# Biomedical-Imaging-Group/MolecularDiffusion_MiViT

Measured on AMD Instinct MI355X. Metric: training image-sequences/sec, higher is better.
Workload: dtype bf16; 1 GPU; PSFNoise 32-frame 64x64 sequences, MiViT depth=4 dim=128 heads=4 hidden=256, linear frame embedding + regression token; train step = fwd + MSE + bwd + AdamW; per_gpu_batch=16384, global_batch=16384, frames=32, frame=64x64, parallelism=dp1, input_dtype=f32 frames resident in HBM

## Files before the change

### moleculardiffusion_mivit_amd/csrc/fused_bwd.hip

```cpp
#include "common.h"
#include "stream_prims.h"
#include <stdlib.h>
#include <algorithm>
#include <vector>
#include <stdio.h>
#include <type_traits>
#include "elem.h"

#define RC(call) do { int rc_ = (call); if (rc_) return rc_; } while (0)

namespace {

#ifdef MIVIT_WIDTH64
constexpr int E = 64, F = 128;
constexpr int LDE = E + 16, LDF = F + 16;
#else
constexpr int E = 128, F = 256;
constexpr int LDE = E + 16, LDF = F + 16;
#endif
constexpr int NW = 4, NT = NW * 64, R = 32;
constexpr int KS = E / 32, ET = E / 16;
constexpr int CPR = E / 8;
constexpr int RPP = NT / CPR, RPT = R / RPP;
constexpr int FW = F / NW, NTW = FW / 16;
// ... 242 lines not shown
#pragma unroll
                for (int nt = 0; nt < NTW; ++nt) {
                    dW1[nt][t] = mma(dhB[nt], xb, dW1[nt][t]);
                    dW2[t][nt] = mma(zb, hB[nt], dW2[t][nt]);
                }
                xb = xn; zb = zn;
            }
        }
        PT_MARK(4);
        barrier();
        PT_MARK(5);
        f32x4 dx[KT2][2];
#pragma unroll
        for (int kt = 0; kt < KT2; ++kt)
#pragma unroll
            for (int rt = 0; rt < 2; ++rt) dx[kt][rt] = zero;
        {
            auto wfrag = [&](int ks, int kt) {
                return tr_pair(W1i + (32 * ks + 4 * g + q) * LDE + EW * wave + 16 * kt + 4 * pp,
                               W1i + (32 * ks + 16 + 4 * g + q) * LDE + EW * wave + 16 * kt + 4 * pp);
            };
            const bf16 *dbase[2] = {DH + (4 * g + q) * R + ((g & 1) << 4) + 4 * pp, DH + (4 * g + q) * R + (((g & 1) ^ 1) << 4) + 4 * pp};
            auto dfrag = [&](int ks, int rt) { return tr_pair(dbase[rt] + 32 * ks * R, dbase[rt] + (32 * ks + 16) * R); };
            bf16x8 d0 = dfrag(0, 0), d1 = dfrag(0, 1);
            bf16x8 wf[KT2];
#pragma unroll
            for (int kt = 0; kt < KT2; ++kt) wf[kt] = wfrag(0, kt);
#pragma unroll
            for (int ks = 0; ks < FS; ++ks) {
                bf16x8 e0 = d0, e1 = d1, vf[KT2];
#pragma unroll
                for (int kt = 0; kt < KT2; ++kt) vf[kt] = wf[kt];
                if (ks < FS - 1) {
                    e0 = dfrag(ks + 1, 0); e1 = dfrag(ks + 1, 1);
#pragma unroll
                    for (int kt = 0; kt < KT2; ++kt) vf[kt] = wfrag(ks + 1, kt);
                }
#pragma unroll
                for (int kt = 0; kt < KT2; ++kt) { dx[kt][0] = mma(wf[kt], d0, dx[kt][0]); dx[kt][1] = mma(wf[kt], d1, dx[kt][1]); }
                d0 = e0; d1 = e1;
#pragma unroll
                for (int kt = 0; kt < KT2; ++kt) wf[kt] = vf[kt];
            }
        }
#pragma unroll
        for (int rt = 0; rt < 2; ++rt) {
            const int row = row0 + 16 * rt + cq;
#pragma unroll
            for (int kt = 0; kt < KT2; ++kt) {
                const int col = EW * wave + 16 * kt + 4 * g;
                const uint2 zr = *reinterpret_cast<const uint2 *>(DZ + (16 * rt + cq) * LDE + col);
                f32x4 o = dx[kt][rt];
                o[0] += elem_lo(zr.x); o[1] += elem_hi(zr.x);
                o[2] += elem_lo(zr.y); o[3] += elem_hi(zr.y);
                if (row < a.M) {
                    typedef __attribute__((ext_vector_type(4))) __bf16 bf16x4;
                    const bf16x4 ob = {(__bf16)o[0], (__bf16)o[1], (__bf16)o[2], (__bf16)o[3]};
                    *reinterpret_cast<bf16x4 *>(a.dx1 + (int64_t)row * E + col) = ob;
                }
            }
        }
        PT_MARK(6);
        barrier();
        PT_MARK(7);
    }
#ifdef MIVIT_PHASE_TIMING
    if (a.dbg && lane == 0)
        for (int k = 0; k < 8; ++k) a.dbg[((int64_t)blockIdx.x * NW + wave) * 8 + k] = pt[k];
#endif

    float *sl = a.slabs + (int64_t)blockIdx.x * SL_TOTAL;
#pragma unroll
    for (int nt = 0; nt < NTW; ++nt) {
#pragma unroll
        for (int t = 0; t < ET; ++t)
#pragma unroll
            for (int j = 0; j < 4; ++j) {
                sl[SL_W1 + (FW * wave + 16 * nt + 4 * g + j) * E + 16 * t + cq] = dW1[nt][t][j];
                sl[SL_W2 + (16 * t + 4 * g + j) * F + FW * wave + 16 * nt + cq] = dW2[t][nt][j];
            }
        const float s = x4_sum(db1[nt]);
        if (g == 0) sl[SL_B1 + FW * wave + 16 * nt + cq] = s;
    }
    __syncthreads();
    for (int i = tid; i < 3 * E; i += NT) {
        const int which = i / E, col = i - which * E, cc = col >> 3, e = col & 7;
        float s = 0.f;
        for (int rr = 0; rr < RPP; ++rr) s += cacc[(2 * which + (e >> 2)) * NT + cc + CPR * rr][e & 3];
        sl[(which == 0 ? SL_G2 : which == 1 ? SL_BE2 : SL_B2) + col] = s;
    }
}

#ifndef MIVIT_WIDTH64
constexpr int NW8 = 8, NT8 = NW8 * 64, NH = NT8 / 2;

template <int ACT>
__global__ __launch_bounds__(NT8) void mlp_block_bwd8_kernel(const MlpBwdArgs a) {
    extern __shared__ __attribute__((aligned(16))) unsigned char smem[];
    bf16 *W1i = reinterpret_cast<bf16 *>(smem + OFF_W1);
    bf16 *X = reinterpret_cast<bf16 *>(smem + OFF_X), *DZ = reinterpret_cast<bf16 *>(smem + OFF_DZ), *DH = reinterpret_cast<bf16 *>(smem + OFF_DH);
    float *b1f = reinterpret_cast<float *>(smem + OFF_VEC);
    f32x4 *cacc = reinterpret_cast<f32x4 *>(smem + OFF_ACC);
    uint4 *stg = reinterpret_cast<uint4 *>(smem + OFF_STG);
    float *rst = reinterpret_cast<float *>(smem + OFF_RST);
    const int tid = threadIdx.x, lane = tid & 63, wave = tid >> 6, g = lane >> 4, cq = lane & 15, q = cq >> 2, pp = cq & 3;
    const f32x4 zero = {0.f, 0.f, 0.f, 0.f};
    const int wave_u = __builtin_amdgcn_readfirstlane(wave);
    const bool ew = wave_u < 4;
    const int th = tid & (NH - 1), wh = wave_u & 3;
    const unsigned stg_a = __builtin_amdgcn_readfirstlane(lds_addr(stg)) + wh * 1024u, rst_a = __builtin_amdgcn_readfirstlane(lds_addr(rst)) + wh * 256u;

    static_assert((F * (E / 8)) % (4 * NT8) == 0, "W1 staging batches");
    for (int i0 = tid; i0 < F * (E / 8); i0 += 4 * NT8) {
        uint4 v0, v1, v2, v3;
        {
            const int i = i0, n = i / (E / 8), cc = i - n * (E / 8);
            v0 = *reinterpret_cast<const uint4 *>(a.W1 + (int64_t)n * E + cc * 8);
        }
        { const int i = i0 + NT8, n = i / (E / 8), cc = i - n * (E / 8); v1 = *reinterpret_cast<const uint4 *>(a.W1 + (int64_t)n * E + cc * 8); }
        { const int i = i0 + 2 * NT8, n = i / (E / 8), cc = i - n * (E / 8); v2 = *reinterpret_cast<const uint4 *>(a.W1 + (int64_t)n * E + cc * 8); }
        { const int i = i0 + 3 * NT8, n = i / (E / 8), cc = i - n * (E / 8); v3 = *reinterpret_cast<const uint4 *>(a.W1 + (int64_t)n * E + cc * 8); }
        { const int i = i0, n = i / (E / 8), cc = i - n * (E / 8); *reinterpret_cast<uint4 *>(W1i + n * LDE + cc * 8) = v0; }
        { const int i = i0 + NT8, n = i / (E / 8), cc = i - n * (E / 8); *reinterpret_cast<uint4 *>(W1i + n * LDE + cc * 8) = v1; }
        { const int i = i0 + 2 * NT8, n = i / (E / 8), cc = i - n * (E / 8); *reinterpret_cast<uint4 *>(W1i + n * LDE + cc * 8) = v2; }
        { const int i = i0 + 3 * NT8, n = i / (E / 8), cc = i - n * (E / 8); *reinterpret_cast<uint4 *>(W1i + n * LDE + cc * 8) = v3; }
    }
    for (int n = tid; n < F; n += NT8) b1f[n] = a.b1[n];
    for (int i = tid; i < E; i += NT8) { b1f[F + i] = a.gamma2[i]; b1f[F + E + i] = a.gamma1[i]; b1f[F + 2 * E + i] = a.beta1[i]; }
    bf16x8 w2f[2][4];
#pragma unroll
    for (int nt = 0; nt < 2; ++nt) {
        const int n = 32 * wave + 16 * nt + cq;
#pragma unroll
        for (int ks = 0; ks < 4; ++ks) {
            bf16x8 t;
#pragma unroll
            for (int e = 0; e < 8; ++e) t[e] = __builtin_bit_cast(__bf16, a.W2[(int64_t)(ks * 32 + 8 * g + e) * F + n].v);
            w2f[nt][ks] = t;
        }
    }
    typedef __attribute__((address_space(3))) const float lds_cf;
    if (ew) {
#pragma unroll
        for (int i = 0; i < 6; ++i) cacc[i * NH + th] = f32x4{0.f, 0.f, 0.f, 0.f};
    }
    f32x4 dW1[2][8], dW2[8][2];
#pragma unroll
    for (int i = 0; i < 2; ++i)
#pragma unroll
        for (int j = 0; j < 8; ++j) { dW1[i][j] = zero; dW2[j][i] = zero; }
    float db1[2] = {0.f, 0.f};
    __syncthreads();

    const int ntiles = (a.M + R - 1) / R;
    int tile = blockIdx.x;
    auto prefetch = [&](int t, int r0, int c) {
#pragma unroll
        for (int i = 0; i < 2; ++i) {
            const int row = min(t * R + r0 + 16 * i, a.M - 1);
            const unsigned o = ((unsigned)row * E + 8 * c) * 2u;
            if (ew) {
                dma16_sbase(a.dy, o, stg_a + (2 * i + 0) * NH * 16u);
                dma16_sbase(a.n2, o, stg_a + (2 * i + 1) * NH * 16u);
                dma4_sbase(a.rstd2, (unsigned)row * 4u, rst_a + i * NH * 4u);
            } else {
                dma16_sbase(a.n1, o, stg_a + (4 + i) * NH * 16u);
            }
        }
    };
    if (tile < ntiles) prefetch(tile, th >> 4, th & 15);
    bool first = true;
#ifdef MIVIT_PHASE_TIMING
    unsigned long long pt[8] = {0, 0, 0, 0, 0, 0, 0, 0}, pt_last = __builtin_amdgcn_s_memtime();
#endif
    for (; tile < ntiles; tile += gridDim.x) {
        const int row0 = tile * R;
        int thv = th;
        asm volatile("" : "+v"(thv));
        const int c = thv & 15, r0 = thv >> 4;
        lds_cf *gam2 = (lds_cf *)(b1f + F + 8 * c), *gam1 = (lds_cf *)(b1f + F + E + 8 * c), *bet1 = (lds_cf *)(b1f + F + 2 * E + 8 * c);
        if (first) wait_vm<0>(); else wait_vm<2>();
        first = false;
        PT_MARK(0);
        if (ew) {
            float sg[8], sb[8], sz[8];
#pragma unroll
            for (int e = 0; e < 8; ++e) sg[e] = sb[e] = sz[e] = 0.f;
            typedef __attribute__((address_space(3))) const f32x4 lds_cf4;
            const f32x4 g2a = *(lds_cf4 *)(gam2), g2b = *(lds_cf4 *)(gam2 + 4);
            const float g2v[8] = {g2a[0], g2a[1], g2a[2], g2a[3], g2b[0], g2b[1], g2b[2], g2b[3]};
#pragma unroll
            for (int i = 0; i < 2; ++i) {
                float d[8], nh[8];
                const bool ok = row0 + r0 + 16 * i < a.M;
                const uint4 pdy = keep_if(stg[(2 * i + 0) * NH + thv], ok), pn2 = stg[(2 * i + 1) * NH + thv];
                unpack8(pdy, d); unpack8(pn2, nh);
                float s1 = 0.f, s2 = 0.f;
#pragma unroll
                for (int e = 0; e < 8; ++e) {
                    sg[e] += d[e] * nh[e]; sb[e] += d[e];
                    d[e] *= g2v[e];
                    s1 += d[e]; s2 += d[e] * nh[e];
                }
                s1 = g16_sum(s1) * (1.f / E); s2 = g16_sum(s2) * (1.f / E);
                const float prs = __uint_as_float(__float_as_uint(rst[i * NH + thv]) & (ok ? 0xffffffffu : 0u));
                float dz[8];
#pragma unroll
                for (int e = 0; e < 8; ++e) { dz[e] = prs * (d[e] - s1 - nh[e] * s2); sz[e] += dz[e]; }
                store16(DZ + (r0 + 16 * i) * LDE + 8 * c, dz);
                __builtin_amdgcn_sched_barrier(0);
            }
            {
                f32x4 ca[3];
#pragma unroll
                for (int k = 0; k < 3; ++k) ca[k] = cacc[k * NH + thv];
                __builtin_amdgcn_sched_barrier(0);
                cacc[0 * NH + thv] = ca[0] + f32x4{sg[0], sg[1], sg[2], sg[3]}; cacc[1 * NH + thv] = ca[1] + f32x4{sg[4], sg[5], sg[6], sg[7]};
                cacc[2 * NH + thv] = ca[2] + f32x4{sb[0], sb[1], sb[2], sb[3]};
                __builtin_amdgcn_sched_barrier(0);
#pragma unroll
                for (int k = 0; k < 3; ++k) ca[k] = cacc[(3 + k) * NH + thv];
                __builtin_amdgcn_sched_barrier(0);
                cacc[3 * NH + thv] = ca[0] + f32x4{sb[4], sb[5], sb[6], sb[7]};
                cacc[4 * NH + thv] = ca[1] + f32x4{sz[0], sz[1], sz[2], sz[3]}; cacc[5 * NH + thv] = ca[2] + f32x4{sz[4], sz[5], sz[6], sz[7]};
            }
        } else {
            typedef __attribute__((address_space(3))) const f32x4 lds_cf4;
            const f32x4 g1a = *(lds_cf4 *)(gam1), g1b = *(lds_cf4 *)(gam1 + 4), b1a = *(lds_cf4 *)(bet1), b1b = *(lds_cf4 *)(bet1 + 4);
            const float g1v[8] = {g1a[0], g1a[1], g1a[2], g1a[3], g1b[0], g1b[1], g1b[2], g1b[3]};
            const float b1v[8] = {b1a[0], b1a[1], b1a[2], b1a[3], b1b[0], b1b[1], b1b[2], b1b[3]};
#pragma unroll
            for (int i = 0; i < 2; ++i) {
                const bool ok = row0 + r0 + 16 * i < a.M;
                const uint4 pn1 = keep_if(stg[(4 + i) * NH + thv], ok);
                float x1v[8];
                unpack8(pn1, x1v);
#pragma unroll
                for (int e = 0; e < 8; ++e) x1v[e] = ok ? x1v[e] * g1v[e] + b1v[e] : 0.f;
                store16(X + (r0 + 16 * i) * LDE + 8 * c, x1v);
            }
        }
        asm volatile("s_waitcnt lgkmcnt(0)" ::: "memory");
        PT_MARK(1);
        prefetch(min(tile + (int)gridDim.x, ntiles - 1), r0, c);
        barrier();
        PT_MARK(2);
        bf16x8 hB[2], dhB[2];
        {
            typedef __attribute__((ext_vector_type(4))) __bf16 bf16x4;
            const int dst_lane = (32 * wave + cq) * R + 4 * g, dst_sw0 = (q & 1) << 4, dst_sw1 = ((q & 1) ^ 1) << 4;
            bf16x4 hlo[2], dlo[2];
#pragma unroll
            for (int rt = 0; rt < 2; ++rt) {
                f32x4 u[2], dh[2];
#pragma unroll
                for (int n2 = 0; n2 < 2; ++n2) {
                    const float bv = b1f[32 * wave + 16 * n2 + cq];
                    u[n2] = f32x4{bv, bv, bv, bv}; dh[n2] = zero;
                }
#pragma unroll
                for (int ks = 0; ks < 4; ++ks) {
                    const bf16x8 xa = lds_frag(X + (16 * rt + cq) * LDE + ks * 32 + 8 * g);
                    const bf16x8 za = lds_frag(DZ + (16 * rt + cq) * LDE + ks * 32 + 8 * g);
#pragma unroll
                    for (int n2 = 0; n2 < 2; ++n2) {
                        u[n2] = mma(xa, lds_frag(W1i + (32 * wave + 16 * n2 + cq) * LDE + ks * 32 + 8 * g), u[n2]);
                        dh[n2] = mma(za, w2f[n2][ks], dh[n2]);
                    }
                }
#pragma unroll
                for (int n2 = 0; n2 < 2; ++n2) {
#pragma unroll
                    for (int j = 0; j < 4; ++j) {
                        const float uu = u[n2][j];
                        dh[n2][j] *= act_bwd(ACT, ACT == MIVIT_ACT_GELU ? uu : act_fwd(ACT, uu));
                        u[n2][j] = act_fwd(ACT, uu);
                        db1[n2] += dh[n2][j];
                    }
                    const bf16x4 hb = {(__bf16)u[n2][0], (__bf16)u[n2][1], (__bf16)u[n2][2], (__bf16)u[n2][3]};
                    const bf16x4 db = {(__bf16)dh[n2][0], (__bf16)dh[n2][1], (__bf16)dh[n2][2], (__bf16)dh[n2][3]};
                    *reinterpret_cast<bf16x4 *>(DH + dst_lane + (rt ? dst_sw1 : dst_sw0) + 16 * n2 * R) = db;
                    if (rt == 0) { hlo[n2] = hb; dlo[n2] = db; }
                    else {
                        struct { bf16x4 lo, hi; } ph = {hlo[n2], hb}, pd = {dlo[n2], db};
                        hB[n2] = __builtin_bit_cast(bf16x8, ph);
                        dhB[n2] = __builtin_bit_cast(bf16x8, pd);
                    }
                }
            }
        }
        PT_MARK(3);
        {
            bf16x8 xb = tr_pair(X + (4 * g + q) * LDE + 4 * pp, X + (16 + 4 * g + q) * LDE + 4 * pp);
            bf16x8 zb = tr_pair(DZ + (4 * g + q) * LDE + 4 * pp, DZ + (16 + 4 * g + q) * LDE + 4 * pp);
#pragma unroll
            for (int t = 0; t < 8; ++t) {
                bf16x8 xn = xb, zn = zb;
                if (t < 7) {
                    xn = tr_pair(X + (4 * g + q) * LDE + 16 * (t + 1) + 4 * pp, X + (16 + 4 * g + q) * LDE + 16 * (t + 1) + 4 * pp);
                    zn = tr_pair(DZ + (4 * g + q) * LDE + 16 * (t + 1) + 4 * pp, DZ + (16 + 4 * g + q) * LDE + 16 * (t + 1) + 4 * pp);
                }
#pragma unroll
                for (int nt = 0; nt < 2; ++nt) {
                    dW1[nt][t] = mma(dhB[nt], xb, dW1[nt][t]);
                    dW2[t][nt] = mma(zb, hB[nt], dW2[t][nt]);
                }
                xb = xn; zb = zn;
            }
        }
        PT_MARK(4);
        barrier();
        PT_MARK(5);
        f32x4 dx[2] = {zero, zero};
        {
            auto wfrag = [&](int ks) {
                return tr_pair(W1i + (32 * ks + 4 * g + q) * LDE + 16 * wave + 4 * pp, W1i + (32 * ks + 16 + 4 * g + q) * LDE + 16 * wave + 4 * pp);
            };
            const bf16 *dbase[2] = {DH + (4 * g + q) * R + ((g & 1) << 4) + 4 * pp, DH + (4 * g + q) * R + (((g & 1) ^ 1) << 4) + 4 * pp};
            auto dfrag = [&](int ks, int rt) { return tr_pair(dbase[rt] + 32 * ks * R, dbase[rt] + (32 * ks + 16) * R); };
            bf16x8 d0 = dfrag(0, 0), d1 = dfrag(0, 1), w0 = wfrag(0);
#pragma unroll
            for (int ks = 0; ks < 8; ++ks) {
                bf16x8 e0 = d0, e1 = d1, v0 = w0;
                if (ks < 7) { e0 = dfrag(ks + 1, 0); e1 = dfrag(ks + 1, 1); v0 = wfrag(ks + 1); }
                dx[0] = mma(w0, d0, dx[0]); dx[1] = mma(w0, d1, dx[1]);
                d0 = e0; d1 = e1; w0 = v0;
            }
        }
#pragma unroll
        for (int rt = 0; rt < 2; ++rt) {
            const int row = row0 + 16 * rt + cq, col = 16 * wave + 4 * g;
            const uint2 zr = *reinterpret_cast<const uint2 *>(DZ + (16 * rt + cq) * LDE + col);
            f32x4 o = dx[rt];
            o[0] += elem_lo(zr.x); o[1] += elem_hi(zr.x);
            o[2] += elem_lo(zr.y); o[3] += elem_hi(zr.y);
            if (row < a.M) {
                typedef __attribute__((ext_vector_type(4))) __bf16 bf16x4;
                const bf16x4 ob = {(__bf16)o[0], (__bf16)o[1], (__bf16)o[2], (__bf16)o[3]};
                *reinterpret_cast<bf16x4 *>(a.dx1 + (int64_t)row * E + col) = ob;
            }
        }
        PT_MARK(6);
        barrier();
        PT_MARK(7);
    }
#ifdef MIVIT_PHASE_TIMING
    if (a.dbg && lane == 0)
        for (int kk = 0; kk < 8; ++kk) a.dbg[((int64_t)blockIdx.x * NW8 + wave) * 8 + kk] = pt[kk];
#endif

    float *sl = a.slabs + (int64_t)blockIdx.x * SL_TOTAL;
#pragma unroll
    for (int nt = 0; nt < 2; ++nt) {
#pragma unroll
        for (int t = 0; t < 8; ++t)
#pragma unroll
            for (int j = 0; j < 4; ++j) {
                sl[SL_W1 + (32 * wave + 16 * nt + 4 * g + j) * E + 16 * t + cq] = dW1[nt][t][j];
                sl[SL_W2 + (16 * t + 4 * g + j) * F + 32 * wave + 16 * nt + cq] = dW2[t][nt][j];
            }
        const float sv = x4_sum(db1[nt]);
        if (g == 0) sl[SL_B1 + 32 * wave + 16 * nt + cq] = sv;
    }
    __syncthreads();
    for (int i = tid; i < 3 * E; i += NT8) {
        const int which = i / E, col = i - which * E, cc = col >> 3, e = col & 7;
        float sv = 0.f;
        for (int rr = 0; rr < 16; ++rr) sv += cacc[(2 * which + (e >> 2)) * NH + cc + 16 * rr][e & 3];
        sl[(which == 0 ? SL_G2 : which == 1 ? SL_BE2 : SL_B2) + col] = sv;
    }
}

#endif

constexpr int AO_OFF_DZ = 0, AO_OFF_CT = AO_OFF_DZ + R * LDE * 2, AO_OFF_STG = AO_OFF_CT + R * LDE * 2;
constexpr int AO_OFF_RED = AO_OFF_STG + 3 * RPT * NT * 16;
constexpr int AO_OFF_RST = AO_OFF_RED + NW * 3 * E * 4;
constexpr int AO_LDS = AO_OFF_RST + RPT * NT * 4;
constexpr int AO_SL_W = 0, AO_SL_B = E * E, AO_SL_G = AO_SL_B + E, AO_SL_BE = AO_SL_G + E, AO_SL_TOTAL = AO_SL_BE + E;
struct AttnOutBwdArgs {
    const bf16 *dy, *n1; const float *rstd1, *gamma1;
    const bf16 *ctx, *Wo;
    int M;
    bf16 *dz1, *dctx;
    float *slabs;
};

__global__ __launch_bounds__(NT, 2) void attn_out_bwd_kernel(const AttnOutBwdArgs a) {
    extern __shared__ __attribute__((aligned(16))) unsigned char smem[];
    bf16 *DZ = reinterpret_cast<bf16 *>(smem + AO_OFF_DZ), *CT = reinterpret_cast<bf16 *>(smem + AO_OFF_CT);
    uint4 *stg = reinterpret_cast<uint4 *>(smem + AO_OFF_STG);
    float *red = reinterpret_cast<float *>(smem + AO_OFF_RED);
    float *rst = reinterpret_cast<float *>(smem + AO_OFF_RST);
    const int tid = threadIdx.x, lane = tid & 63, wave = tid >> 6, g = lane >> 4, cq = lane & 15, q = cq >> 2, pp = cq & 3;
    const f32x4 zero = {0.f, 0.f, 0.f, 0.f};
    bf16x8 wof[KT2][KS];
#pragma unroll
    for (int ct = 0; ct < KT2; ++ct)
#pragma unroll
        for (int ks = 0; ks < KS; ++ks) {
            bf16x8 t;
#pragma unroll
            for (int e = 0; e < 8; ++e) t[e] = __builtin_bit_cast(__bf16, a.Wo[(int64_t)(ks * 32 + 8 * g + e) * E + EW * wave + 16 * ct + cq].v);
            wof[ct][ks] = t;
        }
    const int c = tid % CPR, r0 = tid / CPR;
    float gam[8];
#pragma unroll
    for (int e = 0; e < 8; ++e) gam[e] = a.gamma1[8 * c + e];
    float sg[8], sb[8], sz[8];
#pragma unroll
    for (int e = 0; e < 8; ++e) sg[e] = sb[e] = sz[e] = 0.f;
    f32x4 dWo[KT2][ET];
#pragma unroll
    for (int i = 0; i < KT2; ++i)
#pragma unroll
        for (int j = 0; j < ET; ++j) dWo[i][j] = zero;

    const int ntiles = (a.M + R - 1) / R;
    int tile = blockIdx.x;
    auto prefetch = [&](int t) {
#pragma unroll
        for (int i = 0; i < RPT; ++i) {
            const int64_t row = min((int64_t)t * R + r0 + RPP * i, (int64_t)a.M - 1);
            const int64_t o = row * E + 8 * c;
            dma16_opaque(a.dy + o, stg + (3 * i + 0) * NT + wave * 64);
            dma16_opaque(a.n1 + o, stg + (3 * i + 1) * NT + wave * 64);
            dma16_opaque(a.ctx + o, stg + (3 * i + 2) * NT + wave * 64);
            dma4_opaque(a.rstd1 + row, rst + i * NT + wave * 64);
        }
    };
    if (tile < ntiles) prefetch(tile);
    bool first = true;
    for (; tile < ntiles; tile += gridDim.x) {
        const int64_t row0 = (int64_t)tile * R;
        if (first) wait_vm<0>(); else wait_vm<NROWST>();
        first = false;
#pragma unroll
        for (int i = 0; i < RPT; ++i) {
            float d[8], nh[8], gdy[8];
            const bool ok = row0 + r0 + RPP * i < a.M;
            const uint4 pdy = keep_if(stg[(3 * i + 0) * NT + tid], ok), pn = stg[(3 * i + 1) * NT + tid];
            const uint4 pct = keep_if(stg[(3 * i + 2) * NT + tid], ok);
            unpack8(pdy, d); unpack8(pn, nh);
            float s1 = 0.f, s2 = 0.f;
#pragma unroll
            for (int e = 0; e < 8; ++e) {
                gdy[e] = d[e] * gam[e];
                s1 += gdy[e]; s2 += gdy[e] * nh[e];
                sg[e] += d[e] * nh[e]; sb[e] += d[e];
            }
            s1 = g16_sum(s1) * (1.f / E); s2 = g16_sum(s2) * (1.f / E);
            float dz[8];
            const float prs = __uint_as_float(__float_as_uint(rst[i * NT + tid]) & (ok ? 0xffffffffu : 0u));
#pragma unroll
            for (int e = 0; e < 8; ++e) { dz[e] = prs * (gdy[e] - s1 - nh[e] * s2); sz[e] += dz[e]; }
            store16(DZ + (r0 + RPP * i) * LDE + 8 * c, dz);
            if (ok) store16(a.dz1 + (row0 + r0 + RPP * i) * E + 8 * c, dz);
            *reinterpret_cast<uint4 *>(CT + (r0 + RPP * i) * LDE + 8 * c) = pct;
        }
        asm volatile("s_waitcnt lgkmcnt(0)" ::: "memory");
        prefetch(min(tile + (int)gridDim.x, ntiles - 1));
        barrier();
        f32x4 dc[KT2][2];
#pragma unroll
        for (int ct = 0; ct < KT2; ++ct) { dc[ct][0] = zero; dc[ct][1] = zero; }
#pragma unroll
        for (int ks = 0; ks < KS; ++ks) {
            const bf16x8 z0 = lds_frag(DZ + cq * LDE + ks * 32 + 8 * g), z1 = lds_frag(DZ + (16 + cq) * LDE + ks * 32 + 8 * g);
#pragma unroll
            for (int ct = 0; ct < KT2; ++ct) { dc[ct][0] = mma(wof[ct][ks], z0, dc[ct][0]); dc[ct][1] = mma(wof[ct][ks], z1, dc[ct][1]); }
        }
#pragma unroll
        for (int rt = 0; rt < 2; ++rt) {
            const int64_t row = row0 + 16 * rt + cq;
            if (row < a.M) {
#pragma unroll
                for (int ct = 0; ct < KT2; ++ct) {
                    typedef __attribute__((ext_vector_type(4))) __bf16 bf16x4;
                    const f32x4 o = dc[ct][rt];
                    const bf16x4 ob = {(__bf16)o[0], (__bf16)o[1], (__bf16)o[2], (__bf16)o[3]};
                    *reinterpret_cast<bf16x4 *>(a.dctx + row * E + EW * wave + 16 * ct + 4 * g) = ob;
                }
            }
        }
#pragma unroll
        for (int et = 0; et < KT2; ++et) {
            const bf16x8 za = tr_pair(DZ + (4 * g + q) * LDE + EW * wave + 16 * et + 4 * pp, DZ + (16 + 4 * g + q) * LDE + EW * wave + 16 * et + 4 * pp);
#pragma unroll
            for (int ct = 0; ct < ET; ++ct) {
                const bf16x8 cb = tr_pair(CT + (4 * g + q) * LDE + 16 * ct + 4 * pp, CT + (16 + 4 * g + q) * LDE + 16 * ct + 4 * pp);
                dWo[et][ct] = mma(za, cb, dWo[et][ct]);
            }
        }
        barrier();
    }
    float *sl = a.slabs + (int64_t)blockIdx.x * AO_SL_TOTAL;
// ... 92 lines not shown
        asm volatile("s_waitcnt lgkmcnt(0)" ::: "memory");
        prefetch(min(tile + (int)gridDim.x, ntiles - 1));
        barrier();
        f32x4 dc[2] = {zero, zero};
#pragma unroll
        for (int ks = 0; ks < KQ; ++ks) {
            const bf16x8 z0 = lds_frag(DQ + cq * LDQ + ks * 32 + 8 * g), z1 = lds_frag(DQ + (16 + cq) * LDQ + ks * 32 + 8 * g);
            dc[0] = mma(wof[ks], z0, dc[0]);
            dc[1] = mma(wof[ks], z1, dc[1]);
        }
#pragma unroll
        for (int rt = 0; rt < 2; ++rt) {
            const int64_t row = row0 + 16 * rt + cq;
            const uint2 rr = *reinterpret_cast<const uint2 *>(RS + (16 * rt + cq) * LDE + 16 * wave + 4 * g);
            f32x4 o = dc[rt];
            o[0] += elem_lo(rr.x); o[1] += elem_hi(rr.x);
            o[2] += elem_lo(rr.y); o[3] += elem_hi(rr.y);
            if (row < a.M) {
                typedef __attribute__((ext_vector_type(4))) __bf16 bf16x4;
                const bf16x4 ob = {(__bf16)o[0], (__bf16)o[1], (__bf16)o[2], (__bf16)o[3]};
                *reinterpret_cast<bf16x4 *>(a.dx + row * E + 16 * wave + 4 * g) = ob;
            }
        }
        bf16x8 za[3];
#pragma unroll
        for (int nt = 0; nt < 3; ++nt) {
            za[nt] = tr_pair(DQ + (4 * g + q) * LDQ + 48 * wave + 16 * nt + 4 * pp, DQ + (16 + 4 * g + q) * LDQ + 48 * wave + 16 * nt + 4 * pp);
            dbv[nt] = mma(za[nt], ones, dbv[nt]);
        }
#pragma unroll
        for (int ct = 0; ct < ET; ++ct) {
            const bf16x8 cb = tr_pair(X + (4 * g + q) * LDE + 16 * ct + 4 * pp, X + (16 + 4 * g + q) * LDE + 16 * ct + 4 * pp);
#pragma unroll
            for (int nt = 0; nt < 3; ++nt) dW[nt][ct] = mma(za[nt], cb, dW[nt][ct]);
        }
        barrier();
    }
    float *sl = a.slabs + (int64_t)blockIdx.x * QB_SL_TOTAL;
    const bool fix = a.fix_gamma != nullptr;
#pragma unroll
    for (int nt = 0; nt < 3; ++nt) {
#pragma unroll
        for (int ct = 0; ct < ET; ++ct) {
            const float gk = fix ? a.fix_gamma[16 * ct + cq] : 1.f, bk = fix ? a.fix_beta[16 * ct + cq] : 0.f;
#pragma unroll
            for (int j = 0; j < 4; ++j)
                sl[QB_SL_W + (48 * wave + 16 * nt + 4 * g + j) * E + 16 * ct + cq] = fix ? dW[nt][ct][j] * gk + dbv[nt][j] * bk : dW[nt][ct][j];
        }
        if (cq == 0) {
#pragma unroll
            for (int j = 0; j < 4; ++j) sl[QB_SL_B + 48 * wave + 16 * nt + 4 * g + j] = dbv[nt][j];
        }
    }
}

bool aligned16(const void *p) { return (reinterpret_cast<uintptr_t>(p) & 15) == 0; }
int grid_for(int M) { return std::min(256, ceil_div(M, R)); }
int qkv_grid_for(int M) { return std::min(256 * QB_WGPC, ceil_div(M, R)); }

}

size_t qkv_bwd_ws_bytes(int M) { return align_up((size_t)qkv_grid_for(std::max(M, 1)) * QB_SL_TOTAL * sizeof(float), 256); }

int launch_qkv_bwd(const void *dqkv, const void *x, const void *Wqkv, const void *res, int M, void *dx, float *dW, float *db,
                   const float *fix_gamma, const float *fix_beta, void *ws, size_t ws_bytes, hipStream_t s) {
    MIVIT_CHECK(dqkv && x && Wqkv && res && dx && dW && db && ws && M > 0, "qkv_bwd: null pointer / empty problem");
    MIVIT_CHECK(aligned16(dqkv) && aligned16(x) && aligned16(res) && aligned16(dx), "qkv_bwd: pointers must be 16-byte aligned");
    MIVIT_CHECK(ws_bytes >= qkv_bwd_ws_bytes(M), "qkv_bwd: workspace too small");
    QkvBwdArgs a{static_cast<const bf16 *>(dqkv), static_cast<const bf16 *>(x), static_cast<const bf16 *>(Wqkv), static_cast<const bf16 *>(res),
                 M, static_cast<bf16 *>(dx), static_cast<float *>(ws), fix_gamma, fix_gamma ? fix_beta : nullptr};
    MIVIT_CHECK((fix_gamma == nullptr) == (fix_beta == nullptr), "qkv_bwd: the input affine needs both gamma and beta");
    const int grid = qkv_grid_for(M);
    {
        ProfScope prof(s);
        MIVIT_HIP(hipFuncSetAttribute(reinterpret_cast<const void *>(qkv_bwd_kernel), hipFuncAttributeMaxDynamicSharedMemorySize, QB_LDS));
        hipLaunchKernelGGL(qkv_bwd_kernel, dim3(grid), dim3(NTQ), QB_LDS, s, a);
        MIVIT_LAUNCH_CHECK();
    }
    const float *sl = static_cast<const float *>(ws);
    if (db == dW + QB_SL_B) return launch_slab_reduce_strided(sl, grid, QB_SL_TOTAL, QB_SL_TOTAL, dW, s);
    RC(launch_slab_reduce_strided(sl + QB_SL_W, grid, QB_SL_TOTAL, QN * E, dW, s));
    return launch_slab_reduce_strided(sl + QB_SL_B, grid, QB_SL_TOTAL, QN, db, s);
}

#ifdef MIVIT_WIDTH64
static const int g_mlp_bwd_waves = 4;
constexpr int NW8 = 8;
#else
static int g_mlp_bwd_waves = [] { const char *e = getenv("MIVIT_MLP_BWD_WAVES"); return e && atoi(e) == 4 ? 4 : 8; }();
#endif
#if !defined(MIVIT_ELEM_F16) && !defined(MIVIT_WIDTH64)
extern "C" int mivit_mlp_block_bwd_set_waves(int waves) {
    const int old = g_mlp_bwd_waves;
    if (waves == 4 || waves == 8) g_mlp_bwd_waves = waves;
    return old;
}
#endif

size_t mlp_block_bwd_ws_bytes(int M) { return align_up((size_t)grid_for(std::max(M, 1)) * SL_TOTAL * sizeof(float), 256); }

int launch_mlp_block_bwd(const void *dy, const void *n2, const float *rstd2, const float *gamma2, const void *n1,
                         const float *gamma1, const float *beta1, const void *W1, const float *b1, const void *W2, int M, int act,
                         void *dx1, float *dW1, float *db1, float *dW2, float *db2, float *dgamma2, float *dbeta2, void *ws,
                         size_t ws_bytes, hipStream_t s) {
    MIVIT_CHECK(dy && n2 && rstd2 && gamma2 && n1 && gamma1 && beta1 && W1 && b1 && W2 && dx1 && dW1 && db1 && dW2 && db2 &&
                dgamma2 && dbeta2 && ws && M > 0, "mlp_block_bwd: null pointer / empty problem");
    MIVIT_CHECK(aligned16(dy) && aligned16(n2) && aligned16(n1) && aligned16(W1) && aligned16(dx1), "mlp_block_bwd: pointers must be 16-byte aligned");
    MIVIT_CHECK(ws_bytes >= mlp_block_bwd_ws_bytes(M), "mlp_block_bwd: workspace too small");
    MlpBwdArgs a{static_cast<const bf16 *>(dy), static_cast<const bf16 *>(n2), rstd2, gamma2, static_cast<const bf16 *>(n1), gamma1,
                 beta1, static_cast<const bf16 *>(W1), b1, static_cast<const bf16 *>(W2), M, static_cast<bf16 *>(dx1),
                 static_cast<float *>(ws), nullptr};
    const int grid = grid_for(M);
    const int waves = g_mlp_bwd_waves;
    MIVIT_CHECK((int64_t)M * E * 2 < (1ll << 32), "mlp_block_bwd: %d rows exceed the 32-bit byte offsets of the row prefetch", M);
#ifdef MIVIT_PHASE_TIMING
    static unsigned long long *dbg_buf = nullptr;
    if (!dbg_buf) MIVIT_HIP(hipMalloc(&dbg_buf, 256 * NW8 * 8 * sizeof(unsigned long long)));
    a.dbg = dbg_buf;
#endif
    {
        ProfScope prof(s);
#ifdef MIVIT_WIDTH64
#define BWD_LAUNCH8(ACT_) do { } while (0)
#else
#define BWD_LAUNCH8(ACT_)                                                                                        \
    do {                                                                                                         \
        auto kern = mlp_block_bwd8_kernel<ACT_>;                                                                 \
        MIVIT_HIP(hipFuncSetAttribute(reinterpret_cast<const void *>(kern), hipFuncAttributeMaxDynamicSharedMemorySize, LDS_BYTES)); \
        hipLaunchKernelGGL(kern, dim3(grid), dim3(NT8), LDS_BYTES, s, a);                                        \
    } while (0)
#endif
#define BWD_LAUNCH(ACT_)                                                                                         \
    do {                                                                                                         \
        if (waves == 8) {                                                                                        \
            BWD_LAUNCH8(ACT_);                                                                                   \
        } else {                                                                                                 \
            auto kern = mlp_block_bwd_kernel<ACT_>;                                                              \
            MIVIT_HIP(hipFuncSetAttribute(reinterpret_cast<const void *>(kern), hipFuncAttributeMaxDynamicSharedMemorySize, LDS_BYTES)); \
            hipLaunchKernelGGL(kern, dim3(grid), dim3(NT), LDS_BYTES, s, a);                                     \
        }                                                                                                        \
    } while (0)
        switch (act) {
            case MIVIT_ACT_RELU: BWD_LAUNCH(MIVIT_ACT_RELU); break;
            case MIVIT_ACT_LEAKY_RELU: BWD_LAUNCH(MIVIT_ACT_LEAKY_RELU); break;
            case MIVIT_ACT_GELU: BWD_LAUNCH(MIVIT_ACT_GELU); break;
            default: BWD_LAUNCH(MIVIT_ACT_NONE); break;
        }
#undef BWD_LAUNCH
#undef BWD_LAUNCH8
        MIVIT_LAUNCH_CHECK();
    }
#ifdef MIVIT_PHASE_TIMING
    {
        static const char *names[8] = {"wait rows", "element-wise", "prefetch+barrier", "u, dh", "dW1, dW2", "barrier", "dx1 + stores", "barrier"};
        const int nwv = waves == 8 ? NW8 : NW;
        std::vector<unsigned long long> h((size_t)grid * nwv * 8);
        MIVIT_HIP(hipStreamSynchronize(s));
        MIVIT_HIP(hipMemcpy(h.data(), dbg_buf, h.size() * sizeof(unsigned long long), hipMemcpyDeviceToHost));
        const int tiles = ceil_div(M, R);
        double tot = 0;
        for (int k = 0; k < 8; ++k) {
            double sum = 0;
            double sum_ew = 0, sum_xw = 0;
            for (int i = 0; i < grid * nwv; ++i) {
                sum += (double)h[(size_t)i * 8 + k];
                ((i % nwv) < 4 ? sum_ew : sum_xw) += (double)h[(size_t)i * 8 + k];
            }
            if (nwv == 8) fprintf(stderr, "[mlp_block_bwd phases]   waves 0-3 %8.1f   waves 4-7 %8.1f\n", sum_ew / 4 / tiles, sum_xw / 4 / tiles);
            const double per_tile = sum / nwv / tiles;
            tot += per_tile;
            fprintf(stderr, "[mlp_block_bwd phases] %-18s %8.1f cycles/tile\n", names[k], per_tile);
        }
        fprintf(stderr, "[mlp_block_bwd phases] total %8.1f cycles/tile, %d tiles, grid %d\n", tot, tiles, grid);
    }
#endif
    const float *sl = static_cast<const float *>(ws);
    if (db1 == dW1 + SL_B1 && dW2 == dW1 + SL_W2 && db2 == dW1 + SL_B2 && dgamma2 == dW1 + SL_G2 && dbeta2 == dW1 + SL_BE2)
        return launch_slab_reduce_strided(sl, grid, SL_TOTAL, SL_TOTAL, dW1, s);
    struct { int off, n; float *out; } parts[] = {{SL_W1, F * E, dW1}, {SL_W2, E * F, dW2}, {SL_B1, F, db1}, {SL_B2, E, db2},
                                                  {SL_G2, E, dgamma2}, {SL_BE2, E, dbeta2}};
    for (auto &p : parts) RC(launch_slab_reduce_strided(sl + p.off, grid, SL_TOTAL, p.n, p.out, s));
    return 0;
}

#ifndef MIVIT_ELEM_F16
extern "C" size_t mivit_mlp_block_bwd_workspace_bytes(int M) { return mlp_block_bwd_ws_bytes(M); }
extern "C" int mivit_mlp_block_bwd(const void *dy, const void *n2, const float *rstd2, const float *gamma2, const void *n1,
                                   const float *gamma1, const float *beta1, const void *W1_bf16, const float *b1,
                                   const void *W2_bf16, int M, int act, void *dx1, float *dW1, float *db1, float *dW2, float *db2,
                                   float *dgamma2, float *dbeta2, void *workspace, size_t workspace_bytes, void *stream) {
    prof_set_tag(MIVIT_PROF_OP);
    hipStream_t s = static_cast<hipStream_t>(stream);
    return launch_mlp_block_bwd(dy, n2, rstd2, gamma2, n1, gamma1, beta1, W1_bf16, b1, W2_bf16, M, act, dx1, dW1, db1, dW2, db2, dgamma2,
                                dbeta2, workspace, workspace_bytes, s);
}

#endif
size_t attn_out_bwd_ws_bytes(int M) { return align_up((size_t)std::min(512, ceil_div(std::max(M, 1), R)) * AO_SL_TOTAL * sizeof(float), 256); }

int launch_attn_out_bwd(const void *dy, const void *n1, const float *rstd1, const float *gamma1, const void *ctx, const void *Wo, int M,
                        void *dz1, void *dctx, float *dWo, float *dbo, float *dgamma1, float *dbeta1, void *ws, size_t ws_bytes,
                        hipStream_t s) {
    MIVIT_CHECK(dy && n1 && rstd1 && gamma1 && ctx && Wo && dz1 && dctx && dWo && dbo && dgamma1 && dbeta1 && ws && M > 0,
                "attn_out_bwd: null pointer / empty problem");
    MIVIT_CHECK(aligned16(dy) && aligned16(n1) && aligned16(ctx) && aligned16(Wo) && aligned16(dz1) && aligned16(dctx),
                "attn_out_bwd: pointers must be 16-byte aligned");
    MIVIT_CHECK(ws_bytes >= attn_out_bwd_ws_bytes(M), "attn_out_bwd: workspace too small");
    AttnOutBwdArgs a{static_cast<const bf16 *>(dy), static_cast<const bf16 *>(n1), rstd1, gamma1, static_cast<const bf16 *>(ctx),
                     static_cast<const bf16 *>(Wo), M, static_cast<bf16 *>(dz1), static_cast<bf16 *>(dctx), static_cast<float *>(ws)};
    const int grid = std::min(512, ceil_div(M, R));
    {
        ProfScope prof(s);
        MIVIT_HIP(hipFuncSetAttribute(reinterpret_cast<const void *>(attn_out_bwd_kernel), hipFuncAttributeMaxDynamicSharedMemorySize, AO_LDS));
        hipLaunchKernelGGL(attn_out_bwd_kernel, dim3(grid), dim3(NT), AO_LDS, s, a);
        MIVIT_LAUNCH_CHECK();
    }
    const float *sl = static_cast<const float *>(ws);
    if (dbo == dWo + AO_SL_B && dgamma1 == dWo + AO_SL_G && dbeta1 == dWo + AO_SL_BE)
        return launch_slab_reduce_strided(sl, grid, AO_SL_TOTAL, AO_SL_TOTAL, dWo, s);
    struct { int off, n; float *out; } parts[] = {{AO_SL_W, E * E, dWo}, {AO_SL_B, E, dbo}, {AO_SL_G, E, dgamma1}, {AO_SL_BE, E, dbeta1}};
    for (auto &p : parts) RC(launch_slab_reduce_strided(sl + p.off, grid, AO_SL_TOTAL, p.n, p.out, s));
    return 0;
}

#ifndef MIVIT_ELEM_F16
extern "C" size_t mivit_qkv_bwd_workspace_bytes(int M) { return qkv_bwd_ws_bytes(M); }
extern "C" int mivit_qkv_bwd(const void *dqkv, const void *x, const void *Wqkv_bf16, const void *res, int M, void *dx, float *dW, float *db,
                             void *workspace, size_t workspace_bytes, void *stream) {
    prof_set_tag(MIVIT_PROF_OP);
    return launch_qkv_bwd(dqkv, x, Wqkv_bf16, res, M, dx, dW, db, nullptr, nullptr, workspace, workspace_bytes, static_cast<hipStream_t>(stream));
}
extern "C" size_t mivit_attn_out_bwd_workspace_bytes(int M) { return attn_out_bwd_ws_bytes(M); }
extern "C" int mivit_attn_out_bwd(const void *dy, const void *n1, const float *rstd1, const float *gamma1, const void *ctx,
                                  const void *Wo_bf16, int M, void *dz1, void *dctx, float *dWo, float *dbo, float *dgamma1,
                                  float *dbeta1, void *workspace, size_t workspace_bytes, void *stream) {
    prof_set_tag(MIVIT_PROF_OP);
    return launch_attn_out_bwd(dy, n1, rstd1, gamma1, ctx, Wo_bf16, M, dz1, dctx, dWo, dbo, dgamma1, dbeta1, workspace, workspace_bytes,
                               static_cast<hipStream_t>(stream));
}
#endif
```

Baseline: 1.951 million sequences/s.

## Software-pipeline MLP backward: overlap next tile's element-wise phase with dx GEMM

Restructures the 8-wave MLP block backward loop so the element-wise phase (dz for LayerNorm-2 waves, x1 rebuild for the other waves) for the next tile runs in the same barrier interval as the dx1 GEMM of the current tile. One barrier per tile is removed, and the residual dz values are read into registers before the barrier so the DZ buffer can be overwritten. The goal is to shorten per-tile critical path by overlapping work across wave groups. The cost is more register pressure, plus ordering assumptions about LDS buffer reuse (X, DZ, DH) across the reduced barriers.

```diff
diff --git a/moleculardiffusion_mivit_amd/csrc/fused_bwd.hip b/moleculardiffusion_mivit_amd/csrc/fused_bwd.hip
--- a/moleculardiffusion_mivit_amd/csrc/fused_bwd.hip
+++ b/moleculardiffusion_mivit_amd/csrc/fused_bwd.hip
@@ -418,7 +418,7 @@
     float db1[2] = {0.f, 0.f};
     __syncthreads();
 
-    const int ntiles = (a.M + R - 1) / R;
+    const int ntiles = (a.M + R - 1) / R, G = gridDim.x;
     int tile = blockIdx.x;
     auto prefetch = [&](int t, int r0, int c) {
 #pragma unroll
@@ -434,83 +434,128 @@
             }
         }
     };
-    if (tile < ntiles) prefetch(tile, th >> 4, th & 15);
-    bool first = true;
 #ifdef MIVIT_PHASE_TIMING
     unsigned long long pt[8] = {0, 0, 0, 0, 0, 0, 0, 0}, pt_last = __builtin_amdgcn_s_memtime();
 #endif
-    for (; tile < ntiles; tile += gridDim.x) {
-        const int row0 = tile * R;
+    auto dz_phase = [&](int t, int tn) {
         int thv = th;
         asm volatile("" : "+v"(thv));
-        const int c = thv & 15, r0 = thv >> 4;
-        lds_cf *gam2 = (lds_cf *)(b1f + F + 8 * c), *gam1 = (lds_cf *)(b1f + F + E + 8 * c), *bet1 = (lds_cf *)(b1f + F + 2 * E + 8 * c);
-        if (first) wait_vm<0>(); else wait_vm<2>();
-        first = false;
-        PT_MARK(0);
-        if (ew) {
-            float sg[8], sb[8], sz[8];
-#pragma unroll
-            for (int e = 0; e < 8; ++e) sg[e] = sb[e] = sz[e] = 0.f;
-            typedef __attribute__((address_space(3))) const f32x4 lds_cf4;
-            const f32x4 g2a = *(lds_cf4 *)(gam2), g2b = *(lds_cf4 *)(gam2 + 4);
-            const float g2v[8] = {g2a[0], g2a[1], g2a[2], g2a[3], g2b[0], g2b[1], g2b[2], g2b[3]};
-#pragma unroll
-            for (int i = 0; i < 2; ++i) {
-                float d[8], nh[8];
-                const bool ok = row0 + r0 + 16 * i < a.M;
-                const uint4 pdy = keep_if(stg[(2 * i + 0) * NH + thv], ok), pn2 = stg[(2 * i + 1) * NH + thv];
-                unpack8(pdy, d); unpack8(pn2, nh);
-                float s1 = 0.f, s2 = 0.f;
-#pragma unroll
-                for (int e = 0; e < 8; ++e) {
-                    sg[e] += d[e] * nh[e]; sb[e] += d[e];
-                    d[e] *= g2v[e];
-                    s1 += d[e]; s2 += d[e] * nh[e];
-                }
-                s1 = g16_sum(s1) * (1.f / E); s2 = g16_sum(s2) * (1.f / E);
-                const float prs = __uint_as_float(__float_as_uint(rst[i * NH + thv]) & (ok ? 0xffffffffu : 0u));
-                float dz[8];
-#pragma unroll
-                for (int e = 0; e < 8; ++e) { dz[e] = prs * (d[e] - s1 - nh[e] * s2); sz[e] += dz[e]; }
-                store16(DZ + (r0 + 16 * i) * LDE + 8 * c, dz);
-                __builtin_amdgcn_sched_barrier(0);
-            }
-            {
-                f32x4 ca[3];
-#pragma unroll
-                for (int k = 0; k < 3; ++k) ca[k] = cacc[k * NH + thv];
-                __builtin_amdgcn_sched_barrier(0);
-                cacc[0 * NH + thv] = ca[0] + f32x4{sg[0], sg[1], sg[2], sg[3]}; cacc[1 * NH + thv] = ca[1] + f32x4{sg[4], sg[5], sg[6], sg[7]};
-                cacc[2 * NH + thv] = ca[2] + f32x4{sb[0], sb[1], sb[2], sb[3]};
-                __builtin_amdgcn_sched_barrier(0);
-#pragma unroll
-                for (int k = 0; k < 3; ++k) ca[k] = cacc[(3 + k) * NH + thv];
-                __builtin_amdgcn_sched_barrier(0);
-                cacc[3 * NH + thv] = ca[0] + f32x4{sb[4], sb[5], sb[6], sb[7]};
-                cacc[4 * NH + thv] = ca[1] + f32x4{sz[0], sz[1], sz[2], sz[3]}; cacc[5 * NH + thv] = ca[2] + f32x4{sz[4], sz[5], sz[6], sz[7]};
-            }
-        } else {
-            typedef __attribute__((address_space(3))) const f32x4 lds_cf4;
-            const f32x4 g1a = *(lds_cf4 *)(gam1), g1b = *(lds_cf4 *)(gam1 + 4), b1a = *(lds_cf4 *)(bet1), b1b = *(lds_cf4 *)(bet1 + 4);
-            const float g1v[8] = {g1a[0], g1a[1], g1a[2], g1a[3], g1b[0], g1b[1], g1b[2], g1b[3]};
-            const float b1v[8] = {b1a[0], b1a[1], b1a[2], b1a[3], b1b[0], b1b[1], b1b[2], b1b[3]};
-#pragma unroll
-            for (int i = 0; i < 2; ++i) {
-                const bool ok = row0 + r0 + 16 * i < a.M;
-                const uint4 pn1 = keep_if(stg[(4 + i) * NH + thv], ok);
-                float x1v[8];
-                unpack8(pn1, x1v);
-#pragma unroll
-                for (int e = 0; e < 8; ++e) x1v[e] = ok ? x1v[e] * g1v[e] + b1v[e] : 0.f;
-                store16(X + (r0 + 16 * i) * LDE + 8 * c, x1v);
-            }
+        const int c = thv & 15, r0 = thv >> 4, row0 = t * R;
+        lds_cf *gam2 = (lds_cf *)(b1f + F + 8 * c);
+        float sg[8], sb[8], sz[8];
+#pragma unroll
+        for (int e = 0; e < 8; ++e) sg[e] = sb[e] = sz[e] = 0.f;
+        typedef __attribute__((address_space(3))) const f32x4 lds_cf4;
+        const f32x4 g2a = *(lds_cf4 *)(gam2), g2b = *(lds_cf4 *)(gam2 + 4);
+        const float g2v[8] = {g2a[0], g2a[1], g2a[2], g2a[3], g2b[0], g2b[1], g2b[2], g2b[3]};
+#pragma unroll
+        for (int i = 0; i < 2; ++i) {
+            float d[8], nh[8];
+            const bool ok = row0 + r0 + 16 * i < a.M;
+            const uint4 pdy = keep_if(stg[(2 * i + 0) * NH + thv], ok), pn2 = stg[(2 * i + 1) * NH + thv];
+            unpack8(pdy, d); unpack8(pn2, nh);
+            float s1 = 0.f, s2 = 0.f;
+#pragma unroll
+            for (int e = 0; e < 8; ++e) {
+                sg[e] += d[e] * nh[e]; sb[e] += d[e];
+                d[e] *= g2v[e];
+                s1 += d[e]; s2 += d[e] * nh[e];
+            }
+            s1 = g16_sum(s1) * (1.f / E); s2 = g16_sum(s2) * (1.f / E);
+            const float prs = __uint_as_float(__float_as_uint(rst[i * NH + thv]) & (ok ? 0xffffffffu : 0u));
+            float dz[8];
+#pragma unroll
+            for (int e = 0; e < 8; ++e) { dz[e] = prs * (d[e] - s1 - nh[e] * s2); sz[e] += dz[e]; }
+            store16(DZ + (r0 + 16 * i) * LDE + 8 * c, dz);
+            __builtin_amdgcn_sched_barrier(0);
+        }
+        {
+            f32x4 ca[3];
+#pragma unroll
+            for (int k = 0; k < 3; ++k) ca[k] = cacc[k * NH + thv];
+            __builtin_amdgcn_sched_barrier(0);
+            cacc[0 * NH + thv] = ca[0] + f32x4{sg[0], sg[1], sg[2], sg[3]}; cacc[1 * NH + thv] = ca[1] + f32x4{sg[4], sg[5], sg[6], sg[7]};
+            cacc[2 * NH + thv] = ca[2] + f32x4{sb[0], sb[1], sb[2], sb[3]};
+            __builtin_amdgcn_sched_barrier(0);
+#pragma unroll
+            for (int k = 0; k < 3; ++k) ca[k] = cacc[(3 + k) * NH + thv];
+            __builtin_amdgcn_sched_barrier(0);
+            cacc[3 * NH + thv] = ca[0] + f32x4{sb[4], sb[5], sb[6], sb[7]};
+            cacc[4 * NH + thv] = ca[1] + f32x4{sz[0], sz[1], sz[2], sz[3]}; cacc[5 * NH + thv] = ca[2] + f32x4{sz[4], sz[5], sz[6], sz[7]};
         }
         asm volatile("s_waitcnt lgkmcnt(0)" ::: "memory");
-        PT_MARK(1);
-        prefetch(min(tile + (int)gridDim.x, ntiles - 1), r0, c);
+        if (tn < ntiles) prefetch(tn, r0, c);
+    };
+    auto x1_phase = [&](int t, int tn) {
+        int thv = th;
+        asm volatile("" : "+v"(thv));
+        const int c = thv & 15, r0 = thv >> 4, row0 = t * R;
+        lds_cf *gam1 = (lds_cf *)(b1f + F + E + 8 * c), *bet1 = (lds_cf *)(b1f + F + 2 * E + 8 * c);
+        typedef __attribute__((address_space(3))) const f32x4 lds_cf4;
+        const f32x4 g1a = *(lds_cf4 *)(gam1), g1b = *(lds_cf4 *)(gam1 + 4), b1a = *(lds_cf4 *)(bet1), b1b = *(lds_cf4 *)(bet1 + 4);
+        const float g1v[8] = {g1a[0], g1a[1], g1a[2], g1a[3], g1b[0], g1b[1], g1b[2], g1b[3]};
+        const float b1v[8] = {b1a[0], b1a[1], b1a[2], b1a[3], b1b[0], b1b[1], b1b[2], b1b[3]};
+#pragma unroll
+        for (int i = 0; i < 2; ++i) {
+            const bool ok = row0 + r0 + 16 * i < a.M;
+            const uint4 pn1 = keep_if(stg[(4 + i) * NH + thv], ok);
+            float x1v[8];
+            unpack8(pn1, x1v);
+#pragma unroll
+            for (int e = 0; e < 8; ++e) x1v[e] = ok ? x1v[e] * g1v[e] + b1v[e] : 0.f;
+            store16(X + (r0 + 16 * i) * LDE + 8 * c, x1v);
+        }
+        asm volatile("s_waitcnt lgkmcnt(0)" ::: "memory");
+        if (tn < ntiles) prefetch(tn, r0, c);
+    };
+    auto dx_phase = [&](int row0, const uint2 (&zr)[2]) {
+        int lv = lane;
+        asm volatile("" : "+v"(lv));
+        const int g = lv >> 4, cq = lv & 15, q = cq >> 2, pp = cq & 3, wave = wave_u;
+        f32x4 dx[2] = {zero, zero};
+        {
+            auto wfrag = [&](int ks) {
+                return tr_pair(W1i + (32 * ks + 4 * g + q) * LDE + 16 * wave + 4 * pp, W1i + (32 * ks + 16 + 4 * g + q) * LDE + 16 * wave + 4 * pp);
+            };
+            const bf16 *dbase[2] = {DH + (4 * g + q) * R + ((g & 1) << 4) + 4 * pp, DH + (4 * g + q) * R + (((g & 1) ^ 1) << 4) + 4 * pp};
+            auto dfrag = [&](int ks, int rt) { return tr_pair(dbase[rt] + 32 * ks * R, dbase[rt] + (32 * ks + 16) * R); };
+            bf16x8 d0 = dfrag(0, 0), d1 = dfrag(0, 1), w0 = wfrag(0);
+#pragma unroll
+            for (int ks = 0; ks < 8; ++ks) {
+                bf16x8 e0 = d0, e1 = d1, v0 = w0;
+                if (ks < 7) { e0 = dfrag(ks + 1, 0); e1 = dfrag(ks + 1, 1); v0 = wfrag(ks + 1); }
+                dx[0] = mma(w0, d0, dx[0]); dx[1] = mma(w0, d1, dx[1]);
+                d0 = e0; d1 = e1; w0 = v0;
+            }
+        }
+#pragma unroll
+        for (int rt = 0; rt < 2; ++rt) {
+            const int row = row0 + 16 * rt + cq, col = 16 * wave + 4 * g;
+            f32x4 o = dx[rt];
+            o[0] += elem_lo(zr[rt].x); o[1] += elem_hi(zr[rt].x);
+            o[2] += elem_lo(zr[rt].y); o[3] += elem_hi(zr[rt].y);
+            if (row < a.M) {
+                typedef __attribute__((ext_vector_type(4))) __bf16 bf16x4;
+                const bf16x4 ob = {(__bf16)o[0], (__bf16)o[1], (__bf16)o[2], (__bf16)o[3]};
+                *reinterpret_cast<bf16x4 *>(a.dx1 + (int64_t)row * E + col) = ob;
+            }
+        }
+    };
+
+    if (tile < ntiles) {
+        prefetch(tile, th >> 4, th & 15);
+        wait_vm<0>();
+        PT_MARK(3);
+        if (ew) dz_phase(tile, tile + G); else x1_phase(tile, tile + G);
         barrier();
-        PT_MARK(2);
+        PT_MARK(7);
+    }
+    bool first = true;
+    for (; tile < ntiles; tile += G) {
+        const int row0 = tile * R;
+        int lv = lane;
+        asm volatile("" : "+v"(lv));
+        const int g = lv >> 4, cq = lv & 15, q = cq >> 2, pp = cq & 3, wave = wave_u;
         bf16x8 hB[2], dhB[2];
         {
             typedef __attribute__((ext_vector_type(4))) __bf16 bf16x4;
@@ -555,7 +600,8 @@
                 }
             }
         }
-        PT_MARK(3);
+        PT_MARK(0);
+        uint2 zr[2];
         {
             bf16x8 xb = tr_pair(X + (4 * g + q) * LDE + 4 * pp, X + (16 + 4 * g + q) * LDE + 4 * pp);
             bf16x8 zb = tr_pair(DZ + (4 * g + q) * LDE + 4 * pp, DZ + (16 + 4 * g + q) * LDE + 4 * pp);
@@ -573,42 +619,35 @@
                 }
                 xb = xn; zb = zn;
             }
-        }
-        PT_MARK(4);
+#pragma unroll
+            for (int rt = 0; rt < 2; ++rt) zr[rt] = *reinterpret_cast<const uint2 *>(DZ + (16 * rt + cq) * LDE + 16 * wave + 4 * g);
+        }
+        PT_MARK(1);
         barrier();
-        PT_MARK(5);
-        f32x4 dx[2] = {zero, zero};
-        {
-            auto wfrag = [&](int ks) {
-                return tr_pair(W1i + (32 * ks + 4 * g + q) * LDE + 16 * wave + 4 * pp, W1i + (32 * ks + 16 + 4 * g + q) * LDE + 16 * wave + 4 * pp);
-            };
-            const bf16 *dbase[2] = {DH + (4 * g + q) * R + ((g & 1) << 4) + 4 * pp, DH + (4 * g + q) * R + (((g & 1) ^ 1) << 4) + 4 * pp};
-            auto dfrag = [&](int ks, int rt) { return tr_pair(dbase[rt] + 32 * ks * R, dbase[rt] + (32 * ks + 16) * R); };
-            bf16x8 d0 = dfrag(0, 0), d1 = dfrag(0, 1), w0 = wfrag(0);
-#pragma unroll
-            for (int ks = 0; ks < 8; ++ks) {
-                bf16x8 e0 = d0, e1 = d1, v0 = w0;
-                if (ks < 7) { e0 = dfrag(ks + 1, 0); e1 = dfrag(ks + 1, 1); v0 = wfrag(ks + 1); }
-                dx[0] = mma(w0, d0, dx[0]); dx[1] = mma(w0, d1, dx[1]);
-                d0 = e0; d1 = e1; w0 = v0;
-            }
-        }
-#pragma unroll
-        for (int rt = 0; rt < 2; ++rt) {
-            const int row = row0 + 16 * rt + cq, col = 16 * wave + 4 * g;
-            const uint2 zr = *reinterpret_cast<const uint2 *>(DZ + (16 * rt + cq) * LDE + col);
-            f32x4 o = dx[rt];
-            o[0] += elem_lo(zr.x); o[1] += elem_hi(zr.x);
-            o[2] += elem_lo(zr.y); o[3] += elem_hi(zr.y);
-            if (row < a.M) {
-                typedef __attribute__((ext_vector_type(4))) __bf16 bf16x4;
-                const bf16x4 ob = {(__bf16)o[0], (__bf16)o[1], (__bf16)o[2], (__bf16)o[3]};
-                *reinterpret_cast<bf16x4 *>(a.dx1 + (int64_t)row * E + col) = ob;
-            }
-        }
+        PT_MARK(2);
+        const bool more = tile + G < ntiles;
+        if (ew) {
+            dx_phase(row0, zr);
+            PT_MARK(5);
+            if (more) {
+                wait_vm<2>();
+                PT_MARK(3);
+                dz_phase(tile + G, tile + 2 * G);
+                PT_MARK(4);
+            }
+        } else {
+            if (more) {
+                if (first) wait_vm<0>(); else wait_vm<2>();
+                PT_MARK(3);
+                x1_phase(tile + G, tile + 2 * G);
+                PT_MARK(4);
+            }
+            dx_phase(row0, zr);
+            PT_MARK(5);
+        }
+        first = false;
+        barrier();
         PT_MARK(6);
-        barrier();
-        PT_MARK(7);
     }
 #ifdef MIVIT_PHASE_TIMING
     if (a.dbg && lane == 0)
@@ -1007,8 +1046,10 @@
     }
 #ifdef MIVIT_PHASE_TIMING
     {
-        static const char *names[8] = {"wait rows", "element-wise", "prefetch+barrier", "u, dh", "dW1, dW2", "barrier", "dx1 + stores", "barrier"};
+        static const char *names4[8] = {"wait rows", "element-wise", "prefetch+barrier", "u, dh", "dW1, dW2", "barrier", "dx1 + stores", "barrier"};
+        static const char *names8[8] = {"u, dh", "dW1, dW2 + residual", "barrier A", "wait rows", "phase 0 + prefetch", "dx1 + stores", "barrier B", "prologue"};
         const int nwv = waves == 8 ? NW8 : NW;
+        const char *const *names = waves == 8 ? names8 : names4;
         std::vector<unsigned long long> h((size_t)grid * nwv * 8);
         MIVIT_HIP(hipStreamSynchronize(s));
         MIVIT_HIP(hipMemcpy(h.data(), dbg_buf, h.size() * sizeof(unsigned long long), hipMemcpyDeviceToHost));
```

Result: no change. 1.955 million sequences/s (median of 6 runs) (+0.2%).
